# andimarafioti/faster-qwen3-tts

Hardware: AMD Instinct MI355X
Metric: real-time factor (audio s / wall s), Qwen3-TTS-12Hz-0.6B voice-clone streaming chunk_size=8; p50 TTFA in ttfa_ms_p50 (higher is better)
Workload: dtype bf16

## Files before the change

faster-qwen3-tts_amd/csrc/fq3_api.hip:

```cpp
#define FQ3_SKINNY_EXTERN
#include "fq3_ctx.h"
#include "sampler.cuh"
#include "sampler_wave.cuh"
#include "skinny_gemm.cuh"

#include <cstdio>
#include <cstdlib>
#include <cstring>
#include <map>
#include <string>
#include <type_traits>
#include <vector>

using namespace fq3;

static thread_local std::string g_err;
static int fail(int code, const std::string& m) { g_err = m; return code; }
int fq3_fail_(int code, const std::string& m) { return fail(code, m); }
#define HIPCHK(x) do { hipError_t e_ = (x); if (e_ != hipSuccess) return fail(FQ3_EHIP, std::string(#x) + ": " + hipGetErrorString(e_)); } while (0)

extern "C" const char* fq3_last_error(void) { return g_err.c_str(); }
extern "C" void fq3_set_error_(const char* msg) { g_err = msg ? msg : ""; }
extern "C" int fq3_abi_version(void) { return FQ3_ABI_VERSION; }

// ... 184 lines not shown
    const int Vm = std::max(t.vocab, p.vocab);
    const int G = cfg->num_code_groups;
    const int frames = cfg->max_frames > 0 ? cfg->max_frames : 4096;
    c->cfg.max_frames = frames;
    if ((r = dmalloc(c, &c->h, (size_t)Hm * c->esz))) return r;
    if ((r = dmalloc(c, &c->h2, (size_t)Hm * c->esz))) return r;
    if ((r = dmalloc(c, &c->qkv2, (size_t)qkvm * c->esz))) return r;
    if ((r = dmalloc(c, &c->attn_out, (size_t)qkvm * c->esz))) return r;
    if ((r = dmalloc(c, &c->attn_out2, (size_t)qkvm * c->esz))) return r;
    if ((r = dmalloc(c, &c->act2, (size_t)Im * c->esz))) return r;
    if ((r = dmalloc(c, &c->pred_x2, (size_t)p.hidden * c->esz))) return r;
    if ((r = dmalloc(c, &c->xin, (size_t)Hm * c->esz))) return r;
    if ((r = dmalloc(c, &c->tmp_hidden, (size_t)Hm * c->esz))) return r;
    if ((r = dmalloc(c, &c->qkv, (size_t)qkvm * c->esz))) return r;
    if ((r = dmalloc(c, &c->act, (size_t)Im * c->esz))) return r;
    if ((r = dmalloc(c, &c->logits, (size_t)Vm * c->esz))) return r;
    if ((r = dmalloc(c, &c->past_hidden, (size_t)t.hidden * c->esz))) return r;
    if ((r = dmalloc(c, &c->ph_hold, (size_t)t.hidden * c->esz))) return r;
    if ((r = dmalloc(c, &c->pred_in, (size_t)2 * t.hidden * c->esz))) return r;
    if ((r = dmalloc(c, &c->pred_next, (size_t)t.hidden * c->esz))) return r;
    if ((r = dmalloc(c, &c->pred_x, (size_t)p.hidden * c->esz))) return r;
    if ((r = dmalloc(c, &c->plogits, (size_t)(G - 1) * p.vocab * c->esz))) return r;
    const int maxkv = std::max(t.n_kv_heads, p.n_kv_heads);
    c->part_stride = (size_t)maxkv * kMaxWorkers * 4 * kPartStride;
    if ((r = dmalloc(c, (void**)&c->part, 2 * c->part_stride * sizeof(float)))) return r;
    if ((r = dmalloc(c, (void**)&c->rope_now, 2 * 64 * sizeof(float)))) return r;
    if ((r = dmalloc(c, (void**)&c->seen_api, kMaxVocab))) return r;
    if ((r = dmalloc(c, (void**)&c->st, sizeof(DecodeState)))) return r;
    if ((r = dmalloc(c, (void**)&c->seen, kMaxVocab))) return r;
    if ((r = dmalloc(c, (void**)&c->codes, (size_t)(frames + 1) * G * sizeof(int)))) return r;
    if ((r = dmalloc(c, (void**)&c->ids64, (size_t)64 * sizeof(int64_t)))) return r;
    if ((r = dmalloc(c, (void**)&c->d_pemb, (size_t)64 * sizeof(void*)))) return r;
    HIPCHK(hipStreamCreateWithFlags(&c->cap_stream, hipStreamNonBlocking));
    return FQ3_OK;
}

extern "C" int fq3_set_option(fq3_ctx* c, const char* key, int value) {
    if (!c || !key) return fail(FQ3_EINVAL, "null argument");
    const std::string k(key);
    if (k == "weight_nt") c->opt_nt = value;
    else if (k == "pred_m2") c->opt_m2 = value;
    else if (k == "pred_attn") c->opt_pred_attn = value;
    else if (k == "rows_per_wave_max") c->opt_rmax = value;
    else if (k == "prefill_mode") c->prefill_mode = value;
    else if (k == "flash_prefill") c->opt_flash_prefill = value;
    else if (k == "flash_small") c->opt_flash_small = value;
    else if (k == "cont_pack") c->opt_cont_pack = value;
    else if (k == "swiglu_tile") c->opt_swiglu_tile = value;
    else if (k == "packed_weights") c->opt_packed = value;
    else if (k == "skinny_gemm") c->opt_no_skinny = !value;
    else return fail(FQ3_EINVAL, "unknown option: " + k);
    fq3_graph_reset(c);
    return FQ3_OK;
}

extern "C" int fq3_graph_reset(fq3_ctx* c) {
    if (!c) return fail(FQ3_EINVAL, "null ctx");
    if (c->exec) { (void)hipGraphExecDestroy(c->exec); c->exec = nullptr; }
    if (c->graph) { (void)hipGraphDestroy(c->graph); c->graph = nullptr; }
    return FQ3_OK;
}

namespace {
struct PackedEntry { void* p; int refs; int N, K; };
std::mutex g_packed_mu;
std::map<std::pair<const void*, int>, PackedEntry> g_packed;
// ... 31 lines not shown
}
static int packed_acquire_all(fq3_ctx* c) {
    if (c->cfg.dtype != FQ3_BF16) return FQ3_OK;
    auto take = [&](const void* W, int N, int K, int kind) -> int {
        const int r = fq3_packed_acquire_(W, N, K, kind);
        if (r == FQ3_OK) c->packed_refs.emplace_back(W, kind);
        return r == FQ3_EUNSUPPORTED ? FQ3_OK : r;
    };
    auto stack = [&](const std::vector<fq3_layer_weights>& L, const fq3_stack_dims& d) -> int {
        const int qd = d.n_heads * kHeadDim, kvd = d.n_kv_heads * kHeadDim;
        for (const fq3_layer_weights& l : L) {
            if (int r = take(l.qkv, qd + 2 * kvd, d.hidden, 0)) return r;
            if (int r = take(l.o, d.hidden, qd, 0)) return r;
            if (int r = take(l.gate_up, 2 * d.inter, d.hidden, 1)) return r;
            if (int r = take(l.gate_up, 2 * d.inter, d.hidden, 0)) return r;
            if (int r = take(l.down, d.hidden, d.inter, 0)) return r;
        }
        return FQ3_OK;
    };
    if (int r = stack(c->tl, c->cfg.talker)) return r;
    if (int r = stack(c->pl, c->cfg.predictor)) return r;
    for (const fq3_layer_weights& l : c->tl) if (int r = take(l.gate_up, 2 * c->cfg.talker.inter, c->cfg.talker.hidden, 2)) return r;
    if (int r = take(c->wt.codec_head, c->cfg.talker.vocab, c->cfg.talker.hidden, 0)) return r;
    for (const void* h : c->lmh) if (int r = take(h, c->cfg.predictor.vocab, c->cfg.predictor.hidden, 0)) return r;
    return FQ3_OK;
}

extern "C" int fq3_ctx_destroy(fq3_ctx* c) {
    if (!c) return FQ3_OK;
    (void)hipDeviceSynchronize();
    fq3_graph_reset(c);
    packed_release_all(c);
    if (c->cap_stream) (void)hipStreamDestroy(c->cap_stream);
    if (fq3_kv_pool* p = c->tk.pool) {
        (void)fq3_kv_release(c, 0);
        bool last;
        { std::lock_guard<std::mutex> lk(p->mu); last = --p->users == 0; }
        if (p->is_private && last) pool_free_(p);
    }
    for (void* p : c->allocs) (void)hipFree(p);
    delete c;
    return FQ3_OK;
}

extern "C" int fq3_bind_weights(fq3_ctx* c, const fq3_weight_table* w) {
    if (!c || !w) return fail(FQ3_EINVAL, "null argument");
    const int G = c->cfg.num_code_groups;
    if (!w->talker_layers || !w->predictor_layers || !w->codec_embedding || !w->codec_head || !w->talker_final_norm ||
        !w->predictor_final_norm || !w->predictor_embeddings || !w->lm_heads || !w->talker_cos || !w->talker_sin ||
        !w->pred_cos || !w->pred_sin)
        return fail(FQ3_EINVAL, "weight table has null entries");
    if (c->cfg.has_projection && !w->proj_w) return fail(FQ3_EINVAL, "has_projection set but proj_w is null");
    if (w->talker_rope_len < c->cfg.max_seq_len || w->pred_rope_len < G + 1)
        return fail(FQ3_EINVAL, "rope tables shorter than the caches");
    c->wt = *w;
    c->tl.assign(w->talker_layers, w->talker_layers + c->cfg.talker.n_layers);
    c->pl.assign(w->predictor_layers, w->predictor_layers + c->cfg.predictor.n_layers);
    c->pemb.assign(w->predictor_embeddings, w->predictor_embeddings + (G - 1));
    c->lmh.assign(w->lm_heads, w->lm_heads + (G - 1));
    for (auto& l : c->tl) if (!l.qkv || !l.o || !l.gate_up || !l.down || !l.input_norm || !l.post_norm || !l.q_norm || !l.k_norm)
        return fail(FQ3_EINVAL, "talker layer has null weights");
    for (auto& l : c->pl) if (!l.qkv || !l.o || !l.gate_up || !l.down || !l.input_norm || !l.post_norm || !l.q_norm || !l.k_norm)
        return fail(FQ3_EINVAL, "predictor layer has null weights");
    HIPCHK(hipMemcpy(c->d_pemb, c->pemb.data(), (G - 1) * sizeof(void*), hipMemcpyHostToDevice));
    (void)hipDeviceSynchronize();
    packed_release_all(c);
// ... 799 lines not shown
        if (c->exec) { HIPCHK(hipGraphLaunch(c->exec, s)); }
        else if (int r = enqueue_frame(c, s)) return r;
    }
    LAUNCH_CHECK();
    return FQ3_OK;
}

extern "C" int fq3_decode_poll(fq3_ctx* c, int* n_frames_total, int* done, void* stream) {
    if (!c) return fail(FQ3_EINVAL, "null ctx");
    hipStream_t s = (hipStream_t)stream;
    DecodeState h;
    HIPCHK(hipMemcpyAsync(&h, c->st, sizeof h, hipMemcpyDeviceToHost, s));
    HIPCHK(hipStreamSynchronize(s));
    if (n_frames_total) *n_frames_total = h.frame;
    if (done) *done = h.done == 2 ? 2 : (h.done || h.token == h.eos_id);
    return FQ3_OK;
}

__global__ void codes_to_i64_kernel(const int* src, int64_t* dst, int n) {
    const int i = blockIdx.x * blockDim.x + threadIdx.x;
    if (i < n) dst[i] = src[i];
}

extern "C" int fq3_decode_codes(fq3_ctx* c, int from, int count, int64_t* out, void* stream) {
    if (!c || !out) return fail(FQ3_EINVAL, "null argument");
    if (from < 0 || count < 0 || from + count > c->cfg.max_frames) return fail(FQ3_EINVAL, "range");
    const int G = c->cfg.num_code_groups, n = count * G;
    if (n == 0) return FQ3_OK;
    hipLaunchKernelGGL(codes_to_i64_kernel, dim3((n + 255) / 256), dim3(256), 0, (hipStream_t)stream,
                       c->codes + (size_t)from * G, out, n);
    LAUNCH_CHECK();
    return FQ3_OK;
}
```

faster-qwen3-tts_amd/csrc/fq3_ctx.h:

```cpp
#pragma once
#include "../../include/fq3hip.h"
#include "decode_kernels.cuh"
#include <hip/hip_runtime.h>
#include <mutex>
#include <string>
#include <utility>
#include <vector>

struct fq3_kv_pool {
    int dtype = 0, esz = 2, n_layers = 0, n_kv = 0, n_blocks = 0;
    size_t blk_elems = 0;
    std::vector<void*> k, v;
    std::vector<int> free_list;
    std::mutex mu;
    int in_use_high = 0;
    int users = 0;
    bool is_private = false;
};

struct StackBufs {
    std::vector<void*> k, v;
    int max_seq = 0, workers = 1;
    fq3_kv_pool* pool = nullptr;
    int* d_table = nullptr;
    std::vector<int> blocks;
    int max_blocks = 0;
};

struct fq3_ctx {
    fq3_config cfg{};
    int esz = 2;
    std::vector<fq3_layer_weights> tl, pl;
    fq3_weight_table wt{};
    std::vector<const void*> pemb, lmh;
    const void** d_pemb = nullptr;
    bool bound = false;
    StackBufs tk, pk;
    void *h = nullptr, *xin = nullptr, *qkv = nullptr, *act = nullptr, *logits = nullptr, *past_hidden = nullptr;
    void *pred_in = nullptr, *pred_x = nullptr, *pred_next = nullptr, *plogits = nullptr, *tmp_hidden = nullptr;
    void *attn_out = nullptr, *attn_out2 = nullptr;
    void *h2 = nullptr, *qkv2 = nullptr, *act2 = nullptr, *pred_x2 = nullptr;
    size_t part_stride = 0;
    float* part = nullptr;
    float* rope_now = nullptr;
    unsigned char* seen_api = nullptr;
    fq3::DecodeState* st = nullptr;
    fq3::TeacherForcing* tf = nullptr;
    unsigned char* seen = nullptr;
    int* codes = nullptr;
    int64_t* ids64 = nullptr;
    int n_pad = 0, rope_delta = 0;
    int opt_nt = 1;
    int opt_m2 = 1;
    int opt_pred_attn = 1;
    int opt_rmax = 2;
    int opt_flash_prefill = 1;
    int opt_flash_small = 1;
    int opt_cont_pack = 1;
    int opt_swiglu_tile = 1;
    int opt_packed = 1;
    std::vector<std::pair<const void*, int>> packed_refs;
    int opt_no_skinny = 0;
    int prefill_mode = 0;
    bool talker_wave = true;
    fq3_sampling pred_sampling{0.9f, 50, 1.0f, 1, 1.0f};
    hipGraph_t graph = nullptr;
    hipGraphExec_t exec = nullptr;
    hipStream_t cap_stream = nullptr;
    std::vector<void*> allocs;
    fq3_prompt_weights pw{};
    bool pw_bound = false;
    void *pw_x = nullptr, *pw_h = nullptr;
    int pw_cap = 0;
    void* ph_hold = nullptr;
    void *tt_tab = nullptr, *tt_x = nullptr, *tt_h = nullptr;
    int tt_alloc = 0;
    int tt_cap = 0, tt_rows = 0;
    bool tt_open = false, tt_session = false;
    bool armed = false;
    const void* begin_trailing = nullptr; int begin_trailing_len = 0;
    void *pf_x = nullptr, *pf_xn = nullptr, *pf_qkv = nullptr, *pf_att = nullptr, *pf_gu = nullptr, *pf_act = nullptr, *pf_ws = nullptr;
};


const void* fq3_packed_find_(const void* W, int kind);
int fq3_packed_acquire_(const void* W, int N, int K, int kind);
void fq3_packed_release_(const void* W, int kind);

int fq3_fail_(int code, const std::string& m);
int fq3_kv_ensure_(fq3_ctx* c, int n_pos, hipStream_t s);
int fq3_prefill_reserve_(fq3_ctx* c);
int fq3_prefill_mfma_(fq3_ctx* c, const void* embeds, int L, int n_pad, void* out_logits, void* out_hidden, hipStream_t s);
int fq3_prefill_continue_mfma_(fq3_ctx* c, const void* embeds, int start, int n, void* out_logits, void* out_hidden, hipStream_t s);
int fq3_prefill_continue_batch_mfma_(fq3_ctx* const* cs, int n, const void* const* embeds, const int* start, const int* cnt,
                                     void* const* out_logits, void* const* out_hidden, hipStream_t s);
int fq3_prefill_batch_mfma_(fq3_ctx* const* cs, int n, const void* const* embeds, const int* L, const int* n_pad, void* const* out_logits,
                            void* const* out_hidden, hipStream_t s);
int fq3_codec_head_launch_(fq3_ctx* c, const void* hidden, void* out_logits, hipStream_t s);
int fq3_dmalloc_(fq3_ctx* c, void** p, size_t bytes);
void fq3_text_project_launch_(fq3_ctx* c, const int64_t* ids, int n, void* x, void* h, void* out, hipStream_t s);
```

faster-qwen3-tts_amd/fq3hip/_lib.py:

```python
from __future__ import annotations

import ctypes as C
import os

import torch

_HERE = os.path.dirname(os.path.abspath(__file__))
LIB_PATH = os.path.join(os.path.dirname(_HERE), "lib", "libfq3hip.so")

FQ3_BF16, FQ3_F32, FQ3_BF16X2 = 0, 1, 2
FQ3_PCM_F32, FQ3_PCM_S16, FQ3_PCM_MULAW, FQ3_PCM_ALAW = 0, 1, 2, 3
FQ3_OK, FQ3_EINVAL, FQ3_EHIP, FQ3_ESTATE, FQ3_ETOOLONG, FQ3_EUNSUPPORTED, FQ3_ENOMEM = 0, -1, -2, -3, -4, -5, -6

vp = C.c_void_p
i32 = C.c_int32


class StackDims(C.Structure):
    _fields_ = [("hidden", i32), ("inter", i32), ("n_layers", i32), ("n_heads", i32), ("n_kv_heads", i32),
                ("head_dim", i32), ("vocab", i32), ("rms_eps", C.c_float)]


class Config(C.Structure):
    _fields_ = [("dtype", i32), ("talker", StackDims), ("predictor", StackDims), ("num_code_groups", i32),
# ... 75 lines not shown
    "fq3_kv_pool_stats": (C.c_int, [vp, C.POINTER(C.c_int), C.POINTER(C.c_int), C.POINTER(C.c_int), C.POINTER(C.c_int64)]),
    "fq3_ctx_create_pooled": (C.c_int, [C.POINTER(Config), vp, C.POINTER(vp)]),
    "fq3_kv_reserve": (C.c_int, [vp, C.c_int, vp]),
    "fq3_kv_release": (C.c_int, [vp, C.c_int]),
    "fq3_kv_blocks": (C.c_int, [vp]),
    "fq3_bind_weights": (C.c_int, [vp, C.POINTER(WeightTable)]),
    "fq3_set_option": (C.c_int, [vp, C.c_char_p, C.c_int]),
    "fq3_kv_import": (C.c_int, [vp, C.c_int, vp, vp, C.c_int, vp]),
    "fq3_kv_export": (C.c_int, [vp, C.c_int, vp, vp, C.c_int, vp]),
    "fq3_kv_adopt": (C.c_int, [vp, vp, C.c_int, vp]),
    "fq3_kv_copy": (C.c_int, [vp, vp, C.c_int, vp]),
    "fq3_set_generation_state": (C.c_int, [vp, C.c_int, C.c_int]),
    "fq3_talker_step": (C.c_int, [vp, vp, C.c_int, vp, vp]),
    "fq3_prefill": (C.c_int, [vp, vp, C.c_int, C.c_int, vp, vp, vp]),
    "fq3_prefill_continue": (C.c_int, [vp, vp, C.c_int, C.c_int, vp, vp, vp]),
    "fq3_prefill_reserve": (C.c_int, [vp]),
    "fq3_prefill_continue_batch": (C.c_int, [C.POINTER(vp), C.c_int, C.POINTER(vp), C.POINTER(C.c_int), C.POINTER(C.c_int), C.POINTER(vp),
                                             C.POINTER(vp), vp]),
    "fq3_prefill_batch": (C.c_int, [C.POINTER(vp), C.c_int, C.POINTER(vp), C.POINTER(C.c_int), C.POINTER(C.c_int), C.POINTER(vp),
                                    C.POINTER(vp), vp]),
    "fq3_set_prefill_mode": (C.c_int, [vp, C.c_int]),
    "fq3_codec_head": (C.c_int, [vp, vp, vp, vp]),
    "fq3_set_predictor_sampling": (C.c_int, [vp, C.POINTER(Sampling)]),
    "fq3_predictor_loop": (C.c_int, [vp, vp, vp, vp, vp, vp]),
    "fq3_sample": (C.c_int, [vp, vp, C.c_int, C.POINTER(Sampling), vp, C.c_int, C.c_int, C.c_int, C.c_int,
                             C.c_int, vp, vp, vp]),
    "fq3_apply_repetition_penalty": (C.c_int, [vp, vp, C.c_int, vp, C.c_int, C.c_float, vp]),
    "fq3_decode_begin": (C.c_int, [vp, C.POINTER(DecodeParams), vp]),
    "fq3_decode_cancel": (C.c_int, [vp, vp]),
    "fq3_decode_set_forced": (C.c_int, [vp, vp, vp, vp]),
    "fq3_decode_frames": (C.c_int, [vp, C.c_int, vp]),
    "fq3_decode_poll": (C.c_int, [vp, C.POINTER(C.c_int), C.POINTER(C.c_int), vp]),
    "fq3_decode_codes": (C.c_int, [vp, C.c_int, C.c_int, vp, vp]),
    "fq3_graph_capture": (C.c_int, [vp, vp]),
    "fq3_graph_reset": (C.c_int, [vp]),
    "fq3_bind_prompt_weights": (C.c_int, [vp, C.POINTER(PromptWeights)]),
    "fq3_text_project": (C.c_int, [vp, vp, C.c_int, vp, vp]),
    "fq3_decode_text_open": (C.c_int, [vp, C.c_int, vp]),
    "fq3_decode_text_append": (C.c_int, [vp, vp, C.c_int, C.c_int, vp]),
    "fq3_decode_text_rows": (C.c_int, [vp, C.POINTER(C.c_int), C.POINTER(C.c_int)]),
    "fq3_decode_text_read": (C.c_int, [vp, C.c_int, C.c_int, vp, vp]),
    "fq3_prompt_rows": (C.c_int, [vp, vp, C.c_int, vp, C.c_int, vp, C.c_int, vp, vp, vp]),
    "fq3_batch_create": (C.c_int, [C.POINTER(vp), C.c_int, C.POINTER(vp)]),
    "fq3_batch_destroy": (C.c_int, [vp]),
    "fq3_batch_size": (C.c_int, [vp]),
    "fq3_batch_frames": (C.c_int, [vp, C.c_int, vp]),
    "fq3_batch_graph_capture": (C.c_int, [vp, vp]),
    "fq3_batch_graph_reset": (C.c_int, [vp]),
    "fq3_batch_set_option": (C.c_int, [vp, C.c_char_p, C.c_int]),
    "fq3_batch_set_group_streams": (C.c_int, [vp, C.POINTER(vp), C.c_int]),
    "fq3_batch_poll_async": (C.c_int, [vp, C.c_int, vp]),
    "fq3_batch_poll_wait": (C.c_int, [vp, C.c_int, C.POINTER(C.c_int), C.POINTER(C.c_int)]),
    "fq3_batch_text_append": (C.c_int, [vp, C.c_int, C.POINTER(C.c_int32), C.POINTER(C.c_int32), C.POINTER(C.c_int32), vp, vp]),
    "fq3_codec_create": (C.c_int, [C.POINTER(CodecConfig), C.POINTER(vp)]),
    "fq3_codec_destroy": (C.c_int, [vp]),
    "fq3_codec_set_option": (C.c_int, [vp, C.c_char_p, C.c_int]),
    "fq3_codec_bind": (C.c_int, [vp, C.c_char_p, vp, C.c_int64]),
    "fq3_codec_finalize": (C.c_int, [vp, vp]),
    "fq3_codec_num_samples": (C.c_int64, [vp, C.c_int]),
    "fq3_codec_decode": (C.c_int, [vp, vp, C.c_int, vp, vp]),
    "fq3_codec_decode_tail": (C.c_int, [vp, vp, C.c_int, C.c_int64, vp, vp]),
    "fq3_codec_decode_batch": (C.c_int, [vp, vp, C.c_int, C.c_int, C.c_int64, vp, vp]),
    "fq3_codec_prefix_create": (C.c_int, [vp, vp, C.c_int, C.POINTER(vp), vp]),
    "fq3_codec_prefix_destroy": (C.c_int, [vp]),
    "fq3_codec_prefix_frames": (C.c_int, [vp]),
    "fq3_codec_decode_batch_prefix": (C.c_int, [vp, C.POINTER(vp), vp, C.c_int, C.c_int, C.c_int64, vp, vp]),
# ... 69 lines not shown
```

faster-qwen3-tts_amd/fq3hip/engine.py:

```python
from __future__ import annotations

import ctypes as C
import threading
from typing import Dict, Optional

import torch

from . import _lib as L
from .config import TTSConfig, StackConfig

Weights = Dict[str, torch.Tensor]
_CAPTURE_LOCK = threading.Lock()


def _ptr(t: Optional[torch.Tensor]) -> Optional[int]:
    return None if t is None else t.data_ptr()


def rope_tables(head_dim: int, theta: float, n_pos: int, dtype: torch.dtype):
    inv = 1.0 / (theta ** (torch.arange(0, head_dim, 2, dtype=torch.float) / head_dim))
    ang = torch.arange(n_pos, dtype=torch.float32)[:, None] * inv[None, :]
    return ang.cos().to(dtype).float().contiguous(), ang.sin().to(dtype).float().contiguous()


# ... 449 lines not shown
        L.check(self.lib.fq3_decode_poll(self.ctx, C.byref(n), C.byref(d), self._stream()))
        return n.value, int(d.value)

    def decode_text_open(self, capacity_rows: int):
        L.check(self.lib.fq3_decode_text_open(self.ctx, int(capacity_rows), self._stream()))

    def decode_text_append(self, ids, final: bool = False):
        if isinstance(ids, torch.Tensor):
            t = ids.reshape(-1).to(device=self.device, dtype=torch.long).contiguous()
        else:
            t = torch.tensor([int(i) for i in ids], dtype=torch.long, device=self.device)
        n = int(t.numel())
        L.check(self.lib.fq3_decode_text_append(self.ctx, t.data_ptr() if n else None, n, int(bool(final)), self._stream()))
        self._text_ids_keep = t

    def decode_text_rows(self):
        n, c = C.c_int(0), C.c_int(0)
        L.check(self.lib.fq3_decode_text_rows(self.ctx, C.byref(n), C.byref(c)))
        return n.value, bool(c.value)

    def decode_text_read(self, start: int = 0, count: Optional[int] = None) -> torch.Tensor:
        if count is None:
            count = self.decode_text_rows()[0] - int(start)
        out = self.new(int(count), self.cfg.talker.hidden_size)
        L.check(self.lib.fq3_decode_text_read(self.ctx, int(start), int(count), out.data_ptr(), self._stream()))
        return out

    def decode_codes(self, start: int, count: int) -> torch.Tensor:
        out = torch.empty(count, self.cfg.num_code_groups, dtype=torch.long, device=self.device)
        if count:
            L.check(self.lib.fq3_decode_codes(self.ctx, int(start), int(count), out.data_ptr(), self._stream()))
        return out

    def close(self):
        if getattr(self, "ctx", None) and self.ctx.value:
            self.lib.fq3_ctx_destroy(self.ctx)
            self.ctx = L.vp()

    def __del__(self):
        try:
            self.close()
        except Exception:
            pass


class Fq3Batch:

    def __init__(self, lanes):
        lanes = list(lanes)
        if not 1 <= len(lanes) <= 128:
            raise ValueError("a batch holds 1..128 lanes")
        self.lanes = lanes
        self.lib = lanes[0].lib
        self.device = lanes[0].device
        arr = (L.vp * len(lanes))(*[e.ctx.value for e in lanes])
        self.handle = L.vp()
        with torch.cuda.device(self.device):
            L.check(self.lib.fq3_batch_create(arr, len(lanes), C.byref(self.handle)))

    def __len__(self):
        return len(self.lanes)

    def _stream(self) -> int:
        return torch.cuda.current_stream(self.device).cuda_stream

    def frames(self, n: int):
# ... 57 lines not shown
```

faster-qwen3-tts_amd/fq3hip/generate.py:

```python
from __future__ import annotations

import numbers
import time
from typing import Optional, Tuple

import torch

from .predictor_graph import PredictorGraph
from .talker_graph import TalkerGraph

NOISE_RING = 64


def validate_seed(seed):
    if seed is None:
        return None
    if isinstance(seed, bool) or not isinstance(seed, numbers.Integral):
        raise ValueError(f"seed must be an integer in [0, 2**64) or None, got {type(seed).__name__}")
    seed = int(seed)
    if not 0 <= seed < 2 ** 64:
        raise ValueError(f"seed must be in [0, 2**64), got {seed}")
    return seed


def expand_seeds(seeds, n: int):
    if seeds is None:
        return [None] * n
    if isinstance(seeds, (list, tuple)):
        if len(seeds) != n:
            raise ValueError(f"seeds: {len(seeds)} entries for {n} utterances")
        return [validate_seed(s) for s in seeds]
    s = validate_seed(seeds)
    return [(s + i) % 2 ** 64 for i in range(n)]


def _refill(engine, talker_noise, pred_noise, seed=None, first_frame=0):
    if seed is not None:
        if talker_noise is not None or pred_noise is not None:
            engine.noise_fill(talker_noise, pred_noise, seed, first_frame)
        return
    if talker_noise is not None:
        talker_noise.exponential_(1)
    if pred_noise is not None:
        pred_noise.exponential_(1)
# ... 115 lines not shown

def _prefill_and_arm(talker, talker_input_embeds, attention_mask, trailing_text_hiddens, tts_pad_embed, config,
                     predictor_graph, talker_graph, max_new_tokens, min_new_tokens, temperature, top_k, top_p,
                     do_sample, repetition_penalty, use_graph, cache=None, seed=None):
    token, hidden, n_rows, n_pad = _prefill_first_token(talker_graph.engine, talker_input_embeds, attention_mask, config,
                                                        min_new_tokens, temperature, top_k, top_p, do_sample, cache=cache, seed=seed)
    return _arm_decode(talker, config, token, hidden, n_rows, attention_mask, trailing_text_hiddens, tts_pad_embed, predictor_graph,
                       talker_graph, max_new_tokens, min_new_tokens, temperature, top_k, top_p, do_sample, repetition_penalty,
                       use_graph, n_pad=n_pad, seed=seed)


def run_frames(eng, tn, pn, issued: int, count: int, seed=None):
    while count > 0:
        if issued % NOISE_RING == 0:
            if seed is None:
                _refill(eng, tn, pn)
            else:
                _refill(eng, tn, pn, seed, issued)
        k = min(count, NOISE_RING - issued % NOISE_RING)
        eng.decode_frames(k)
        issued += k
        count -= k
    return issued


@torch.inference_mode()
def fast_generate(talker, talker_input_embeds: torch.Tensor, attention_mask: torch.Tensor,
                  trailing_text_hiddens: torch.Tensor, tts_pad_embed: torch.Tensor, config,
                  predictor_graph: PredictorGraph, talker_graph: TalkerGraph, max_new_tokens: int = 2048,
                  min_new_tokens: int = 2, temperature: float = 0.9, top_k: int = 50, top_p: float = 1.0,
                  do_sample: bool = True, repetition_penalty: float = 1.05,
                  subtalker_dosample: Optional[bool] = None, subtalker_top_k: Optional[int] = None,
                  subtalker_top_p: Optional[float] = None, subtalker_temperature: Optional[float] = None,
                  parity_mode: bool = False, poll_every: int = 8, seed: Optional[int] = None) -> Tuple[Optional[torch.Tensor], dict]:
    seed = validate_seed(seed)
    t_start = time.time()
    eng, tn, pn, max_frames = _prefill_and_arm(
        talker, talker_input_embeds, attention_mask, trailing_text_hiddens, tts_pad_embed, config, predictor_graph,
        talker_graph, max_new_tokens, min_new_tokens, temperature, top_k, top_p, do_sample, repetition_penalty,
        use_graph=not parity_mode, seed=seed)
    torch.cuda.current_stream(eng.device).synchronize()
    t_prefill = time.time() - t_start
    t_decode_start = time.time()
    issued, n, done = 0, 0, False
    while not done and issued < max_frames:
        issued = run_frames(eng, tn, pn, issued, min(poll_every, max_frames - issued), seed)
        n, done = eng.decode_poll()
    codes = eng.decode_codes(0, n) if n > 0 else None
    torch.cuda.current_stream(eng.device).synchronize()
    t_decode = time.time() - t_decode_start
    timing = {
        "prefill_ms": t_prefill * 1000,
        "decode_s": t_decode,
        "steps": n,
        "ms_per_step": (t_decode / n * 1000) if n > 0 else 0,
        "steps_per_s": (n / t_decode) if t_decode > 0 else 0,
    }
    return codes, timing
```

faster-qwen3-tts_amd/fq3hip/model.py:

```python
from __future__ import annotations

import contextlib
import logging
import time
from pathlib import Path
from typing import Any, Dict, Generator, List, Optional, Tuple, Union

import numpy as np
import torch

logger = logging.getLogger(__name__)

_GGML_ONLY = ("ref_spk", "ref_rvq", "ref_spk_emb", "ref_codes")


def expand_seeds(seeds, n: int) -> list:
    from .generate import expand_seeds as expand
    return expand(seeds, n)


def _to_numpy(a) -> np.ndarray:
    if hasattr(a, "cpu"):
        return a.flatten().float().cpu().numpy()
    return a.flatten() if hasattr(a, "flatten") else a
# ... 721 lines not shown
                        self.model._tokenize_texts([self.model._build_instruct_text(instruct)])[0]]
        m = self.model.model
        tie, tam, tth, tpe = self._build_talker_inputs_local(
            m=m, input_ids=input_ids, ref_ids=[None], voice_clone_prompt=None,
            languages=[language] if language is not None else ["Auto"], speakers=[speaker],
            non_streaming_mode=non_streaming_mode, instruct_ids=instruct_ids)
        talker, config = self._after_prepare(m, tie)
        return m, talker, config, tie, tam, tth, tpe

    @contextlib.contextmanager
    def audio_output(self, sample_rate: Optional[int] = None, encoding: str = "f32", speed: float = 1.0):
        from .audio_out import AudioOutSpec
        spec = AudioOutSpec(sample_rate, encoding, speed).validate(self.sample_rate)
        prev, self._audio_spec = getattr(self, "_audio_spec", None), spec
        try:
            yield spec
        finally:
            self._audio_spec = prev

    @contextlib.contextmanager
    def seeded(self, seed: Optional[int]):
        from .generate import validate_seed
        seed = validate_seed(seed)
        prev, self._seed = getattr(self, "_seed", None), seed
        try:
            yield seed
        finally:
            self._seed = prev

    def _seed_kw(self) -> dict:
        seed = getattr(self, "_seed", None)
        return {} if seed is None else dict(seed=seed)

    def _refuse_batch_audio_output(self) -> None:
        if getattr(self, "_audio_spec", None) is not None:
            raise ValueError("the batch entry points decode their audio in groups and do not run the audio output stage: call them outside "
                             "audio_output(), or use the single-stream entry points (the server builds one vocoder per request instead)")

    def _one_shot_output(self, wav) -> Tuple[np.ndarray, int]:
        from .audio_out import AudioOut
        dev = torch.device(self.device) if not isinstance(self.device, torch.device) else self.device
        stage = AudioOut(self._audio_spec, self.sample_rate, wav.device if hasattr(wav, "is_cuda") and wav.is_cuda else dev)
        x = wav.flatten().float() if hasattr(wav, "cpu") else torch.from_numpy(np.ascontiguousarray(wav, dtype=np.float32).reshape(-1))
        out = stage.push_host(x.to(stage.dev), final=True)
        if stage.flac:
            out = np.concatenate([np.frombuffer(stage.header(stage.n_samples), dtype=np.uint8), out])
        return out, stage.out_rate

    @staticmethod
    def _tail_event(voc, timing: Optional[dict]):
        if voc.output is None:
            return None
        tail, sr = voc.flush()
        if len(tail) == 0:
            return None
        t = dict(timing or {})
        t.update(chunk_index=t.get("chunk_index", -1) + 1, chunk_steps=0, prefill_ms=0, decode_ms=0.0, is_final=True)
        t.pop("first_text_ms", None)
        return tail, sr, t

    def _run_full(self, m, talker, config, tie, tam, tth, tpe, ref_codes, gen_kwargs) -> Tuple[list, int]:
        from .generate import fast_generate
        codec_ids, timing = fast_generate(talker=talker, talker_input_embeds=tie, attention_mask=tam,
                                          trailing_text_hiddens=tth, tts_pad_embed=tpe, config=config,
                                          predictor_graph=self.predictor_graph, talker_graph=self.talker_graph,
                                          **gen_kwargs, **self._seed_kw())
        if codec_ids is None:
            logger.warning("Generation returned no tokens")
            if self._audio_spec is not None:
                a, sr = self._one_shot_output(np.zeros(1, dtype=np.float32))
                return [a], sr
            return [np.zeros(1, dtype=np.float32)], self.sample_rate
        codes = torch.cat([ref_codes.to(codec_ids.device), codec_ids], dim=0) if ref_codes is not None else codec_ids
        ref_len = ref_codes.shape[0] if ref_codes is not None else 0
        tok = m.speech_tokenizer
        if ref_len > 0 and hasattr(tok, "decode_tensor") and hasattr(tok, "num_samples_total"):
            cut = int(ref_len / max(codes.shape[0], 1) * tok.num_samples_total(codes.shape[0]))
            pf = tok.prefix_for(ref_codes) if hasattr(tok, "prefix_for") else None
            wav = tok.decode_tensor(codes, cut, prefix=pf) if pf is not None else tok.decode_tensor(codes, cut)
            if self._audio_spec is not None:
                a, sr = self._one_shot_output(wav)
                out = [a]
            else:
                out, sr = [_to_numpy(wav)], tok.sample_rate
        elif self._audio_spec is not None and ref_len == 0 and hasattr(tok, "decode_tensor"):
            a, sr = self._one_shot_output(tok.decode_tensor(codes, 0))
            out = [a]
        else:
            audio_list, sr = tok.decode({"audio_codes": codes.unsqueeze(0)})
            out = []
            for a in audio_list:
                a = _to_numpy(a)
                if ref_len > 0:
                    a = a[int(ref_len / max(codes.shape[0], 1) * len(a)):]
                if self._audio_spec is not None:
                    a, sr = self._one_shot_output(a)
                out.append(a)
        n = timing["steps"]
        total = timing["prefill_ms"] / 1000 + timing["decode_s"]
        logger.info("Generated %.2fs audio in %.2fs (%.1fms/step, RTF: %.2f)", n / 12.5, total, timing["ms_per_step"],
                    (n / 12.5) / total if total > 0 else 0)
        return out, sr

    def _vocoder_stream(self, tok):
        use_side = torch.cuda.is_available() and hasattr(tok, "decode_tensor") and hasattr(tok, "num_samples_total")
        if not use_side:
            return None
        if getattr(self, "_voc_stream", None) is None:
            dev = torch.device(self.device) if not isinstance(self.device, torch.device) else self.device
            prio = getattr(self, "vocoder_stream_priority", None)
            share = getattr(self, "vocoder_cu_share", None)
            if share:
                from .streams import cu_masked_stream
                self._voc_stream = cu_masked_stream(dev, float(share))
                return self._voc_stream
            from .streams import concurrent_stream
            self._voc_stream = concurrent_stream(dev, prio)
        return self._voc_stream

    def streaming_vocoder(self, ref_codes, chunk_size: int, output=None) -> "StreamingVocoder":
        tok = self.model.model.speech_tokenizer
        return StreamingVocoder(tok, ref_codes, chunk_size, self.device, self._vocoder_stream(tok),
                                output=output if output is not None else getattr(self, "_audio_spec", None))

    def _run_streaming(self, m, talker, config, tie, tam, tth, tpe, ref_codes, gen_kwargs, chunk_size: int,
                       parity_mode: bool = False):
        from .streaming import fast_generate_streaming, parity_generate_streaming
        tok = m.speech_tokenizer
        voc = StreamingVocoder(tok, ref_codes, chunk_size, self.device, self._vocoder_stream(tok), output=self._audio_spec)
        fn = parity_generate_streaming if parity_mode else fast_generate_streaming
        stream = fn(talker=talker, talker_input_embeds=tie, attention_mask=tam, trailing_text_hiddens=tth,
                    tts_pad_embed=tpe, config=config, predictor_graph=self.predictor_graph,
                    talker_graph=self.talker_graph, chunk_size=chunk_size, **gen_kwargs, **self._seed_kw())
        timing = None
        for chunk, timing in stream:
            ev = timing.pop("codes_ready_event", None)
            new_audio, sr = voc.push(chunk, ev, final=bool(timing.get("is_final")))
            yield new_audio, sr, timing
        tail = self._tail_event(voc, timing)
        if tail is not None:
            yield tail

    @staticmethod
    def _gen_kwargs(max_new_tokens, min_new_tokens, temperature, top_k, top_p, do_sample, repetition_penalty):
        return dict(max_new_tokens=max_new_tokens, min_new_tokens=min_new_tokens, temperature=temperature,
                    top_k=top_k, top_p=top_p, do_sample=do_sample, repetition_penalty=repetition_penalty)

    @torch.inference_mode()
    def generate_voice_clone(self, text: str, language: str, ref_audio: Optional[Union[str, Path]] = None,
                             ref_text: str = "", max_new_tokens: int = 2048, min_new_tokens: int = 2,
                             temperature: float = 0.9, top_k: int = 50, top_p: float = 1.0, do_sample: bool = True,
                             repetition_penalty: float = 1.05, xvec_only: bool = False,
                             non_streaming_mode: Optional[bool] = None, append_silence: bool = True,
                             instruct: Optional[str] = None, ref_spk: Optional[Union[str, Path]] = None,
                             ref_rvq: Optional[Union[str, Path]] = None, ref_spk_emb: Optional[np.ndarray] = None,
                             ref_codes: Optional[np.ndarray] = None,
                             voice_clone_prompt: Optional[Union[Dict[str, Any], List[Any]]] = None) -> Tuple[list, int]:
        self._reject_ggml_cached_reference_args(ref_spk=ref_spk, ref_rvq=ref_rvq, ref_spk_emb=ref_spk_emb,
                                                ref_codes=ref_codes)
        nsm = self._resolve_non_streaming_mode(non_streaming_mode, default=False)
        m, talker, config, tie, tam, tth, tpe, rc = self._prepare_generation(
            text=text, language=language, ref_audio=ref_audio, ref_text=ref_text, xvec_only=xvec_only,
            non_streaming_mode=nsm, append_silence=append_silence, voice_clone_prompt=voice_clone_prompt,
            instruct=instruct)
        return self._run_full(m, talker, config, tie, tam, tth, tpe, rc,
                              self._gen_kwargs(max_new_tokens, min_new_tokens, temperature, top_k, top_p, do_sample,
# ... 647 lines not shown
```

faster-qwen3-tts_amd/fq3hip/streaming.py:

```python
from __future__ import annotations

import time
from typing import Generator, Tuple

import torch

from .generate import _prefill_and_arm, run_frames, validate_seed
from .predictor_graph import PredictorGraph
from .talker_graph import TalkerGraph


@torch.inference_mode()
def fast_generate_streaming(talker, talker_input_embeds: torch.Tensor, attention_mask: torch.Tensor,
                            trailing_text_hiddens: torch.Tensor, tts_pad_embed: torch.Tensor, config,
                            predictor_graph: PredictorGraph, talker_graph: TalkerGraph, max_new_tokens: int = 2048,
                            min_new_tokens: int = 2, temperature: float = 0.9, top_k: int = 50, top_p: float = 1.0,
                            do_sample: bool = True, repetition_penalty: float = 1.05, chunk_size: int = 12,
                            use_graph: bool = True, seed=None) -> Generator[Tuple[torch.Tensor, dict], None, None]:
    seed = validate_seed(seed)
    t_start = time.time()
    eng, tn, pn, max_frames = _prefill_and_arm(
        talker, talker_input_embeds, attention_mask, trailing_text_hiddens, tts_pad_embed, config, predictor_graph,
        talker_graph, max_new_tokens, min_new_tokens, temperature, top_k, top_p, do_sample, repetition_penalty,
        use_graph=use_graph, seed=seed)
    torch.cuda.current_stream(eng.device).synchronize()
    t_prefill = time.time() - t_start
    issued, emitted, chunk_count, done = 0, 0, 0, False
    chunk_start = time.time()
    issued = run_frames(eng, tn, pn, issued, min(chunk_size, max_frames), seed)
    while True:
        n, done = eng.decode_poll()
        new = n - emitted
        if new <= 0:
            break
        chunk = eng.decode_codes(emitted, new)
        ready = torch.cuda.Event()
        ready.record(torch.cuda.current_stream(eng.device))
        emitted = n
        is_final = new < chunk_size
        more = (not done) and (not is_final) and issued < max_frames
        if more:
            issued = run_frames(eng, tn, pn, issued, min(chunk_size, max_frames - issued), seed)
        yield chunk, {
            "chunk_index": chunk_count,
            "chunk_steps": new,
            "prefill_ms": t_prefill * 1000 if chunk_count == 0 else 0,
            "decode_ms": (time.time() - chunk_start) * 1000,
            "total_steps_so_far": emitted,
            "is_final": is_final,
            "codes_ready_event": ready,
        }
        chunk_count += 1
        chunk_start = time.time()
        if not more:
            break


def parity_generate_streaming(talker, talker_input_embeds, attention_mask, trailing_text_hiddens, tts_pad_embed, config,
                              max_new_tokens: int = 2048, min_new_tokens: int = 2, temperature: float = 0.9,
                              top_k: int = 50, top_p: float = 1.0, do_sample: bool = True,
                              repetition_penalty: float = 1.05, chunk_size: int = 12, predictor_graph=None,
                              talker_graph=None, seed=None):
    if predictor_graph is None or talker_graph is None:
        raise ValueError("parity_generate_streaming needs the graph objects of the HIP context")
    return fast_generate_streaming(talker, talker_input_embeds, attention_mask, trailing_text_hiddens, tts_pad_embed,
                                   config, predictor_graph, talker_graph, max_new_tokens=max_new_tokens,
                                   min_new_tokens=min_new_tokens, temperature=temperature, top_k=top_k, top_p=top_p,
                                   do_sample=do_sample, repetition_penalty=repetition_penalty, chunk_size=chunk_size,
                                   use_graph=False, seed=seed)
```

include/fq3hip.h:

```cpp
#ifndef FQ3HIP_H
#define FQ3HIP_H

#include <stdint.h>

#ifdef __cplusplus
extern "C" {
#endif

#define FQ3_ABI_VERSION 5

enum { FQ3_BF16 = 0, FQ3_F32 = 1,
       FQ3_BF16X2 = 2 };
enum { FQ3_OK = 0, FQ3_EINVAL = -1, FQ3_EHIP = -2, FQ3_ESTATE = -3, FQ3_ETOOLONG = -4, FQ3_EUNSUPPORTED = -5, FQ3_ENOMEM = -6 };

typedef struct fq3_stack_dims {
    int32_t hidden, inter, n_layers, n_heads, n_kv_heads, head_dim, vocab;
    float rms_eps;
} fq3_stack_dims;

typedef struct fq3_config {
    int32_t dtype;
    fq3_stack_dims talker;
    fq3_stack_dims predictor;
    int32_t num_code_groups;
// ... 91 lines not shown
                       void* out_logits, void* stream);


int fq3_sample(fq3_ctx* ctx, const void* logits, int V, const fq3_sampling* s, const int64_t* history,
               int n_hist, int sup_lo, int sup_hi, int keep_id, int suppress_eos, const void* noise,
               int64_t* out_token, void* stream);

int fq3_apply_repetition_penalty(fq3_ctx* ctx, void* logits, int V, const int64_t* history, int n_hist, float penalty,
                                 void* stream);


typedef struct fq3_decode_params {
    fq3_sampling talker;
    int32_t min_new_tokens;
    int32_t max_new_tokens;
    int32_t prefill_len;
    int32_t gen_step;
    int32_t first_token;
    const void* past_hidden;
    const void* trailing_text;
    int32_t trailing_len;
    const void* tts_pad_embed;
    const void* talker_noise;
    const void* pred_noise;
    int32_t noise_frames;
} fq3_decode_params;

int fq3_decode_begin(fq3_ctx* ctx, const fq3_decode_params* p, void* stream);
int fq3_decode_cancel(fq3_ctx* ctx, void* stream);
int fq3_decode_set_forced(fq3_ctx* ctx, const int32_t* forced_codes, int32_t* decisions, void* stream);
int fq3_decode_frames(fq3_ctx* ctx, int n_frames, void* stream);
int fq3_decode_poll(fq3_ctx* ctx, int* n_frames_total, int* done, void* stream);
int fq3_decode_codes(fq3_ctx* ctx, int from, int count, int64_t* out_codes_dev, void* stream);
int fq3_graph_capture(fq3_ctx* ctx, void* stream);
int fq3_graph_reset(fq3_ctx* ctx);

typedef struct fq3_prompt_weights {
    const void* text_embedding;
    const void* fc1_w;
    const void* fc1_b;
    const void* fc2_w;
    const void* fc2_b;
    int32_t text_vocab, text_hidden;
} fq3_prompt_weights;
int fq3_bind_prompt_weights(fq3_ctx* ctx, const fq3_prompt_weights* w);
int fq3_text_project(fq3_ctx* ctx, const int64_t* ids, int n, void* out, void* stream);
int fq3_prompt_rows(fq3_ctx* ctx, const void* text_rows, int n_text, const int32_t* prog, int n_rows,
                    const int64_t* ref_codes, int n_ref, const void* spk_embed, void* out, void* stream);

int fq3_decode_text_open(fq3_ctx* ctx, int capacity_rows, void* stream);
int fq3_decode_text_append(fq3_ctx* ctx, const int64_t* ids, int n, int final, void* stream);
int fq3_decode_text_rows(const fq3_ctx* ctx, int* n_rows, int* closed);
int fq3_decode_text_read(fq3_ctx* ctx, int from, int count, void* out, void* stream);

typedef struct fq3_batch fq3_batch;
int fq3_batch_create(fq3_ctx* const* lanes, int n_lanes, fq3_batch** out);
int fq3_batch_destroy(fq3_batch* b);
int fq3_batch_size(const fq3_batch* b);
int fq3_batch_frames(fq3_batch* b, int n_frames, void* stream);
int fq3_batch_graph_capture(fq3_batch* b, void* stream);
int fq3_batch_graph_reset(fq3_batch* b);
int fq3_batch_poll_async(fq3_batch* b, int slot, void* stream);
int fq3_batch_poll_wait(fq3_batch* b, int slot, int* n_frames_total, int* done);
int fq3_batch_text_append(fq3_batch* b, int n_items, const int32_t* lane, const int32_t* count, const int32_t* final_,
                          const int64_t* ids, void* stream);
int fq3_batch_set_option(fq3_batch* b, const char* key, int value);
// ... 103 lines not shown
```

Baseline: 38.63.

## Run decode frames ahead of host polls using async pinned-memory marks

Adds decode_mark/decode_wait, which copy the decode state into pinned host memory and record an event, so the host can queue more frames before waiting. Streaming and batch generation enqueue up to two extra frames past each chunk boundary before synchronising, so the GPU keeps working while the host handles the previous chunk. It also drops the synchronize after prefill and copies codes into a preallocated buffer. The risk is wasted frames past EOS and extra complexity in the state handling.

```diff
diff --git a/faster-qwen3-tts_amd/csrc/fq3_api.hip b/faster-qwen3-tts_amd/csrc/fq3_api.hip
--- a/faster-qwen3-tts_amd/csrc/fq3_api.hip
+++ b/faster-qwen3-tts_amd/csrc/fq3_api.hip
@@ -240,6 +240,8 @@
     if ((r = dmalloc(c, (void**)&c->ids64, (size_t)64 * sizeof(int64_t)))) return r;
     if ((r = dmalloc(c, (void**)&c->d_pemb, (size_t)64 * sizeof(void*)))) return r;
     HIPCHK(hipStreamCreateWithFlags(&c->cap_stream, hipStreamNonBlocking));
+    HIPCHK(hipHostMalloc((void**)&c->mark_host, kMarkSlots * sizeof(DecodeState), hipHostMallocDefault));
+    for (int i = 0; i < kMarkSlots; ++i) HIPCHK(hipEventCreateWithFlags(&c->mark_ev[i], hipEventDisableTiming));
     return FQ3_OK;
 }
 
@@ -337,6 +339,8 @@
     fq3_graph_reset(c);
     packed_release_all(c);
     if (c->cap_stream) (void)hipStreamDestroy(c->cap_stream);
+    for (int i = 0; i < kMarkSlots; ++i) if (c->mark_ev[i]) (void)hipEventDestroy(c->mark_ev[i]);
+    if (c->mark_host) (void)hipHostFree(c->mark_host);
     if (fq3_kv_pool* p = c->tk.pool) {
         (void)fq3_kv_release(c, 0);
         bool last;
@@ -1202,3 +1206,29 @@
     LAUNCH_CHECK();
     return FQ3_OK;
 }
+
+extern "C" int fq3_decode_mark(fq3_ctx* c, int slot, int from, int count, int64_t* out, void* stream) {
+    const fq3_mark_verdict v = fq3_decode_mark_check_(c != nullptr, slot, from, count, c ? c->cfg.max_frames : 0, out != nullptr);
+    if (v.code) return fail(v.code, v.why);
+    hipStream_t s = (hipStream_t)stream;
+    const int G = c->cfg.num_code_groups, n = count * G;
+    if (n > 0) {
+        hipLaunchKernelGGL(codes_to_i64_kernel, dim3((n + 255) / 256), dim3(256), 0, s, c->codes + (size_t)from * G, out, n);
+        LAUNCH_CHECK();
+    }
+    HIPCHK(hipMemcpyAsync(&c->mark_host[slot], c->st, sizeof(DecodeState), hipMemcpyDeviceToHost, s));
+    HIPCHK(hipEventRecord(c->mark_ev[slot], s));
+    c->mark_armed[slot] = true;
+    return FQ3_OK;
+}
+
+extern "C" int fq3_decode_wait(fq3_ctx* c, int slot, int* n_frames_total, int* done) {
+    const fq3_mark_verdict v = fq3_decode_wait_check_(c != nullptr, slot, c ? c->mark_armed : nullptr);
+    if (v.code) return fail(v.code, v.why);
+    HIPCHK(hipEventSynchronize(c->mark_ev[slot]));
+    c->mark_armed[slot] = false;
+    const DecodeState& h = c->mark_host[slot];
+    if (n_frames_total) *n_frames_total = h.frame;
+    if (done) *done = h.done == 2 ? 2 : (h.done || h.token == h.eos_id);
+    return FQ3_OK;
+}
diff --git a/faster-qwen3-tts_amd/csrc/fq3_ctx.h b/faster-qwen3-tts_amd/csrc/fq3_ctx.h
--- a/faster-qwen3-tts_amd/csrc/fq3_ctx.h
+++ b/faster-qwen3-tts_amd/csrc/fq3_ctx.h
@@ -1,6 +1,7 @@
 #pragma once
 #include "../../include/fq3hip.h"
 #include "decode_kernels.cuh"
+#include "mark_args.h"
 #include <hip/hip_runtime.h>
 #include <mutex>
 #include <string>
@@ -67,6 +68,9 @@
     hipGraph_t graph = nullptr;
     hipGraphExec_t exec = nullptr;
     hipStream_t cap_stream = nullptr;
+    fq3::DecodeState* mark_host = nullptr;
+    hipEvent_t mark_ev[kMarkSlots] = {nullptr, nullptr};
+    bool mark_armed[kMarkSlots] = {false, false};
     std::vector<void*> allocs;
     fq3_prompt_weights pw{};
     bool pw_bound = false;
diff --git a/faster-qwen3-tts_amd/csrc/mark_args.h b/faster-qwen3-tts_amd/csrc/mark_args.h
--- /dev/null
+++ b/faster-qwen3-tts_amd/csrc/mark_args.h
@@ -0,0 +1,24 @@
+#pragma once
+#include "../../include/fq3hip.h"
+
+constexpr int kMarkSlots = 2;
+
+struct fq3_mark_verdict {
+    int code;
+    const char* why;
+};
+
+inline fq3_mark_verdict fq3_decode_mark_check_(bool have_ctx, int slot, int from, int count, int max_frames, bool have_out) {
+    if (!have_ctx) return {FQ3_EINVAL, "decode mark: null ctx"};
+    if (slot < 0 || slot >= kMarkSlots) return {FQ3_EINVAL, "decode mark: slot must be 0 or 1"};
+    if (from < 0 || count < 0 || max_frames < 0 || from > max_frames || count > max_frames - from) return {FQ3_EINVAL, "decode mark: range"};
+    if (count > 0 && !have_out) return {FQ3_EINVAL, "decode mark: out_codes is NULL with count > 0"};
+    return {FQ3_OK, nullptr};
+}
+
+inline fq3_mark_verdict fq3_decode_wait_check_(bool have_ctx, int slot, const bool* armed) {
+    if (!have_ctx) return {FQ3_EINVAL, "decode wait: null ctx"};
+    if (slot < 0 || slot >= kMarkSlots) return {FQ3_EINVAL, "decode wait: slot must be 0 or 1"};
+    if (!armed || !armed[slot]) return {FQ3_ESTATE, "decode wait: no mark was queued in this slot"};
+    return {FQ3_OK, nullptr};
+}
diff --git a/faster-qwen3-tts_amd/fq3hip/_lib.py b/faster-qwen3-tts_amd/fq3hip/_lib.py
--- a/faster-qwen3-tts_amd/fq3hip/_lib.py
+++ b/faster-qwen3-tts_amd/fq3hip/_lib.py
@@ -131,6 +131,8 @@
     "fq3_decode_frames": (C.c_int, [vp, C.c_int, vp]),
     "fq3_decode_poll": (C.c_int, [vp, C.POINTER(C.c_int), C.POINTER(C.c_int), vp]),
     "fq3_decode_codes": (C.c_int, [vp, C.c_int, C.c_int, vp, vp]),
+    "fq3_decode_mark": (C.c_int, [vp, C.c_int, C.c_int, C.c_int, vp, vp]),
+    "fq3_decode_wait": (C.c_int, [vp, C.c_int, C.POINTER(C.c_int), C.POINTER(C.c_int)]),
     "fq3_graph_capture": (C.c_int, [vp, vp]),
     "fq3_graph_reset": (C.c_int, [vp]),
     "fq3_bind_prompt_weights": (C.c_int, [vp, C.POINTER(PromptWeights)]),
diff --git a/faster-qwen3-tts_amd/fq3hip/engine.py b/faster-qwen3-tts_amd/fq3hip/engine.py
--- a/faster-qwen3-tts_amd/fq3hip/engine.py
+++ b/faster-qwen3-tts_amd/fq3hip/engine.py
@@ -505,6 +505,17 @@
             L.check(self.lib.fq3_decode_codes(self.ctx, int(start), int(count), out.data_ptr(), self._stream()))
         return out
 
+    def decode_mark(self, slot: int, start: int, count: int, out: Optional[torch.Tensor]):
+        if count:
+            if out.dtype != torch.long or not out.is_contiguous() or out.shape[0] < count or out.shape[1] != self.cfg.num_code_groups:
+                raise ValueError("decode_mark: out must be a contiguous LongTensor [>= count, num_code_groups]")
+        L.check(self.lib.fq3_decode_mark(self.ctx, int(slot), int(start), int(count), out.data_ptr() if count else None, self._stream()))
+
+    def decode_wait(self, slot: int):
+        n, d = C.c_int(0), C.c_int(0)
+        L.check(self.lib.fq3_decode_wait(self.ctx, int(slot), C.byref(n), C.byref(d)))
+        return n.value, bool(d.value)
+
     def close(self):
         if getattr(self, "ctx", None) and self.ctx.value:
             self.lib.fq3_ctx_destroy(self.ctx)
diff --git a/faster-qwen3-tts_amd/fq3hip/generate.py b/faster-qwen3-tts_amd/fq3hip/generate.py
--- a/faster-qwen3-tts_amd/fq3hip/generate.py
+++ b/faster-qwen3-tts_amd/fq3hip/generate.py
@@ -10,6 +10,13 @@
 from .talker_graph import TalkerGraph
 
 NOISE_RING = 64
+RUN_AHEAD = 2
+
+
+def run_ahead_depth(eng, run_ahead) -> int:
+    if isinstance(run_ahead, bool) or not isinstance(run_ahead, numbers.Integral) or run_ahead < 0:
+        raise ValueError(f"run_ahead must be an integer >= 0, got {run_ahead!r}")
+    return int(run_ahead) if hasattr(eng, "decode_mark") and hasattr(eng, "decode_wait") else 0
 
 
 def validate_seed(seed):
@@ -191,20 +198,29 @@
                   do_sample: bool = True, repetition_penalty: float = 1.05,
                   subtalker_dosample: Optional[bool] = None, subtalker_top_k: Optional[int] = None,
                   subtalker_top_p: Optional[float] = None, subtalker_temperature: Optional[float] = None,
-                  parity_mode: bool = False, poll_every: int = 8, seed: Optional[int] = None) -> Tuple[Optional[torch.Tensor], dict]:
+                  parity_mode: bool = False, poll_every: int = 8, seed: Optional[int] = None,
+                  run_ahead: int = RUN_AHEAD) -> Tuple[Optional[torch.Tensor], dict]:
     seed = validate_seed(seed)
     t_start = time.time()
     eng, tn, pn, max_frames = _prefill_and_arm(
         talker, talker_input_embeds, attention_mask, trailing_text_hiddens, tts_pad_embed, config, predictor_graph,
         talker_graph, max_new_tokens, min_new_tokens, temperature, top_k, top_p, do_sample, repetition_penalty,
         use_graph=not parity_mode, seed=seed)
-    torch.cuda.current_stream(eng.device).synchronize()
     t_prefill = time.time() - t_start
+    R = min(run_ahead_depth(eng, run_ahead), poll_every)
     t_decode_start = time.time()
     issued, n, done = 0, 0, False
-    while not done and issued < max_frames:
-        issued = run_frames(eng, tn, pn, issued, min(poll_every, max_frames - issued), seed)
-        n, done = eng.decode_poll()
+    group_end, polls = 0, 0
+    while not done and group_end < max_frames:
+        group_end += min(poll_every, max_frames - group_end)
+        issued = run_frames(eng, tn, pn, issued, group_end - issued, seed)
+        if R > 0:
+            eng.decode_mark(polls & 1, 0, 0, None)
+            issued = run_frames(eng, tn, pn, issued, min(R, max_frames - issued), seed)
+            n, done = eng.decode_wait(polls & 1)
+            polls += 1
+        else:
+            n, done = eng.decode_poll()
     codes = eng.decode_codes(0, n) if n > 0 else None
     torch.cuda.current_stream(eng.device).synchronize()
     t_decode = time.time() - t_decode_start
diff --git a/faster-qwen3-tts_amd/fq3hip/model.py b/faster-qwen3-tts_amd/fq3hip/model.py
--- a/faster-qwen3-tts_amd/fq3hip/model.py
+++ b/faster-qwen3-tts_amd/fq3hip/model.py
@@ -777,6 +777,10 @@
         seed = getattr(self, "_seed", None)
         return {} if seed is None else dict(seed=seed)
 
+    def _run_ahead_kw(self) -> dict:
+        r = getattr(self, "run_ahead", None)
+        return {} if r is None else dict(run_ahead=r)
+
     def _refuse_batch_audio_output(self) -> None:
         if getattr(self, "_audio_spec", None) is not None:
             raise ValueError("the batch entry points decode their audio in groups and do not run the audio output stage: call them outside "
@@ -809,7 +813,7 @@
         codec_ids, timing = fast_generate(talker=talker, talker_input_embeds=tie, attention_mask=tam,
                                           trailing_text_hiddens=tth, tts_pad_embed=tpe, config=config,
                                           predictor_graph=self.predictor_graph, talker_graph=self.talker_graph,
-                                          **gen_kwargs, **self._seed_kw())
+                                          **gen_kwargs, **self._seed_kw(), **self._run_ahead_kw())
         if codec_ids is None:
             logger.warning("Generation returned no tokens")
             if self._audio_spec is not None:
@@ -876,7 +880,7 @@
         fn = parity_generate_streaming if parity_mode else fast_generate_streaming
         stream = fn(talker=talker, talker_input_embeds=tie, attention_mask=tam, trailing_text_hiddens=tth,
                     tts_pad_embed=tpe, config=config, predictor_graph=self.predictor_graph,
-                    talker_graph=self.talker_graph, chunk_size=chunk_size, **gen_kwargs, **self._seed_kw())
+                    talker_graph=self.talker_graph, chunk_size=chunk_size, **gen_kwargs, **self._seed_kw(), **self._run_ahead_kw())
         timing = None
         for chunk, timing in stream:
             ev = timing.pop("codes_ready_event", None)
diff --git a/faster-qwen3-tts_amd/fq3hip/streaming.py b/faster-qwen3-tts_amd/fq3hip/streaming.py
--- a/faster-qwen3-tts_amd/fq3hip/streaming.py
+++ b/faster-qwen3-tts_amd/fq3hip/streaming.py
@@ -5,7 +5,7 @@
 
 import torch
 
-from .generate import _prefill_and_arm, run_frames, validate_seed
+from .generate import RUN_AHEAD, _prefill_and_arm, run_ahead_depth, run_frames, validate_seed
 from .predictor_graph import PredictorGraph
 from .talker_graph import TalkerGraph
 
@@ -16,31 +16,44 @@
                             predictor_graph: PredictorGraph, talker_graph: TalkerGraph, max_new_tokens: int = 2048,
                             min_new_tokens: int = 2, temperature: float = 0.9, top_k: int = 50, top_p: float = 1.0,
                             do_sample: bool = True, repetition_penalty: float = 1.05, chunk_size: int = 12,
-                            use_graph: bool = True, seed=None) -> Generator[Tuple[torch.Tensor, dict], None, None]:
+                            use_graph: bool = True, seed=None, run_ahead: int = RUN_AHEAD) -> Generator[Tuple[torch.Tensor, dict], None, None]:
     seed = validate_seed(seed)
     t_start = time.time()
     eng, tn, pn, max_frames = _prefill_and_arm(
         talker, talker_input_embeds, attention_mask, trailing_text_hiddens, tts_pad_embed, config, predictor_graph,
         talker_graph, max_new_tokens, min_new_tokens, temperature, top_k, top_p, do_sample, repetition_penalty,
         use_graph=use_graph, seed=seed)
-    torch.cuda.current_stream(eng.device).synchronize()
     t_prefill = time.time() - t_start
+    R = min(run_ahead_depth(eng, run_ahead), chunk_size)
     issued, emitted, chunk_count, done = 0, 0, 0, False
     chunk_start = time.time()
     issued = run_frames(eng, tn, pn, issued, min(chunk_size, max_frames), seed)
+    chunk_end = issued
+    codes = torch.empty(max_frames, eng.cfg.num_code_groups, dtype=torch.long, device=eng.device) if R > 0 else None
     while True:
-        n, done = eng.decode_poll()
+        if R > 0:
+            eng.decode_mark(chunk_count & 1, emitted, chunk_end - emitted, codes[emitted:])
+            ready = torch.cuda.Event()
+            ready.record(torch.cuda.current_stream(eng.device))
+            issued = run_frames(eng, tn, pn, issued, min(R, max_frames - issued), seed)
+            n, done = eng.decode_wait(chunk_count & 1)
+        else:
+            n, done = eng.decode_poll()
         new = n - emitted
         if new <= 0:
             break
-        chunk = eng.decode_codes(emitted, new)
-        ready = torch.cuda.Event()
-        ready.record(torch.cuda.current_stream(eng.device))
+        if R > 0:
+            chunk = codes[emitted:n]
+        else:
+            chunk = eng.decode_codes(emitted, new)
+            ready = torch.cuda.Event()
+            ready.record(torch.cuda.current_stream(eng.device))
         emitted = n
         is_final = new < chunk_size
-        more = (not done) and (not is_final) and issued < max_frames
+        more = (not done) and (not is_final) and chunk_end < max_frames
         if more:
-            issued = run_frames(eng, tn, pn, issued, min(chunk_size, max_frames - issued), seed)
+            chunk_end += min(chunk_size, max_frames - chunk_end)
+            issued = run_frames(eng, tn, pn, issued, chunk_end - issued, seed)
         yield chunk, {
             "chunk_index": chunk_count,
             "chunk_steps": new,
@@ -60,11 +73,11 @@
                               max_new_tokens: int = 2048, min_new_tokens: int = 2, temperature: float = 0.9,
                               top_k: int = 50, top_p: float = 1.0, do_sample: bool = True,
                               repetition_penalty: float = 1.05, chunk_size: int = 12, predictor_graph=None,
-                              talker_graph=None, seed=None):
+                              talker_graph=None, seed=None, run_ahead: int = RUN_AHEAD):
     if predictor_graph is None or talker_graph is None:
         raise ValueError("parity_generate_streaming needs the graph objects of the HIP context")
     return fast_generate_streaming(talker, talker_input_embeds, attention_mask, trailing_text_hiddens, tts_pad_embed,
                                    config, predictor_graph, talker_graph, max_new_tokens=max_new_tokens,
                                    min_new_tokens=min_new_tokens, temperature=temperature, top_k=top_k, top_p=top_p,
                                    do_sample=do_sample, repetition_penalty=repetition_penalty, chunk_size=chunk_size,
-                                   use_graph=False, seed=seed)
+                                   use_graph=False, seed=seed, run_ahead=run_ahead)
diff --git a/include/fq3hip.h b/include/fq3hip.h
--- a/include/fq3hip.h
+++ b/include/fq3hip.h
@@ -147,6 +147,8 @@
 int fq3_decode_frames(fq3_ctx* ctx, int n_frames, void* stream);
 int fq3_decode_poll(fq3_ctx* ctx, int* n_frames_total, int* done, void* stream);
 int fq3_decode_codes(fq3_ctx* ctx, int from, int count, int64_t* out_codes_dev, void* stream);
+int fq3_decode_mark(fq3_ctx* ctx, int slot, int from, int count, int64_t* out_codes_dev, void* stream);
+int fq3_decode_wait(fq3_ctx* ctx, int slot, int* n_frames_total, int* done);
 int fq3_graph_capture(fq3_ctx* ctx, void* stream);
 int fq3_graph_reset(fq3_ctx* ctx);
 
```

Result: faster. 39.12, median of 6 (+1.3%).
